# yassouali/pytorch-segmentation

Hardware: NVIDIA H100
Metric: images/sec DeepLabV3+/ResNet101 513x513 train step (fwd+CE+bwd+SGD) (higher is better)
Workload: dtype bf16

## Files before the change

include/seg_b200.h:

```cpp
#ifndef SEG_B200_H
#define SEG_B200_H

#include <stdint.h>

#ifdef __cplusplus
extern "C" {
#endif

#define SEG_DT_BF16 0
#define SEG_DT_F32 1

#define SEG_IMPL_AUTO 0
#define SEG_IMPL_SIMT 1
#define SEG_IMPL_TC 2

typedef struct seg_conv_desc {
  int32_t N, H, W, C;
  int32_t K;
  int32_t R, S;
  int32_t stride, pad, dil;
  int32_t P, Q;
  int32_t ldx;
  int32_t ldy;
} seg_conv_desc;

typedef struct seg_sync_desc {
  void* const* peers;
  int32_t rank, world, n_max;
  int64_t timeout_clocks;
} seg_sync_desc;

const char* seg_last_error(void);
int seg_version(void);
int seg_device_ok(void);
int64_t seg_launch_count(void);
void seg_launch_count_reset(void);

int seg_conv2d_fwd(const seg_conv_desc* d, const void* x, const void* w_packed, void* y, int y_dtype,
                   const float* bias, float beta, double* stats, const seg_sync_desc* sync, void* sync_ticket,
                   int impl, void* stream);
int seg_conv2d_dgrad(const seg_conv_desc* d, const void* dy, const void* w_packed, void* dx, float beta,
                     int impl, void* stream);
int64_t seg_conv2d_wgrad_workspace_floats(const seg_conv_desc* d, int impl);
int seg_conv2d_wgrad(const seg_conv_desc* d, const void* dy, const void* x, float* dw_packed, float* workspace, int impl,
                     void* stream);

int64_t seg_dwconv_scratch_floats(int C);
int seg_dwconv3x3_fwd(const seg_conv_desc* d, const void* x, const float* w9, void* y, double* stats,
                      const seg_sync_desc* sync, void* sync_ticket, void* stream);
int seg_dwconv3x3_bwd_data(const seg_conv_desc* d, const void* dy, const float* w9, void* dx, float beta, void* stream);
int seg_dwconv3x3_bwd_weight(const seg_conv_desc* d, const void* dy, const void* x, float* dw9, float beta,
                             float* scratch, void* stream);
int seg_dw_pack_weight(const float* w_c133, float* w9, int C, void* stream);
int seg_dw_unpack_wgrad(const float* g9, float* g_c133, int C, float beta, void* stream);

int seg_pack_weight(const float* w_oihw, void* w_packed, int K, int C, int R, int S, int Cpad, void* stream);
int seg_unpack_wgrad(const float* dw_packed, float* g_oihw, int K, int C, int R, int S, int Cpad, float beta,
                     void* stream);
int seg_pack_entry_bytes(void);
int seg_pack_weights_batched(const void* table, int n, int64_t total, void* stream);
int seg_unpack_wgrads_batched(const void* table, int n, int64_t total, float beta, void* stream);
int seg_im2col(const seg_conv_desc* d, const void* x, int x_nchw_f32, void* col, int Kpad, void* stream);

int seg_bn_stats(const void* x, int64_t M, int C, int ldx, double* stats, const seg_sync_desc* sync, void* sync_ticket,
                 void* stream);
// ... 161 lines not shown
```

pytorch-segmentation_b200/csrc/seg_api.cu:

```cuda
#include <stdarg.h>
#include "seg_common.cuh"

namespace seg {

static thread_local char g_err[1024] = "";
std::atomic<long long> g_launches{0};

void set_error(const char* fmt, ...) {
  va_list ap;
  va_start(ap, fmt);
  vsnprintf(g_err, sizeof(g_err), fmt, ap);
  va_end(ap);
}

namespace tc {
bool supported(const seg_conv_desc* d);
int conv_fwd(const seg_conv_desc* d, const void* x, const void* w, void* y, int y_dtype, const float* bias, float beta,
             double* stats, unsigned* stat_ticket, const seg_sync_desc* sync, cudaStream_t stream);
int conv_dgrad(const seg_conv_desc* d, const void* dy, const void* w, void* dx, float beta, cudaStream_t stream);
int conv_wgrad(const seg_conv_desc* d, const void* dy, const void* x, float* dw, float* ws, cudaStream_t stream);
int64_t wgrad_workspace_floats(const seg_conv_desc* d);
}
namespace simt {
int conv_fwd(const seg_conv_desc* d, const void* x, const void* w, void* y, int y_dtype, const float* bias, float beta,
             double* stats, unsigned* stat_ticket, const seg_sync_desc* sync, cudaStream_t stream);
int conv_dgrad(const seg_conv_desc* d, const void* dy, const void* w, void* dx, float beta, cudaStream_t stream);
int conv_wgrad(const seg_conv_desc* d, const void* dy, const void* x, float* dw, cudaStream_t stream);
}

static int check_desc(const seg_conv_desc* d) {
  SEG_REQUIRE(d != nullptr, "null conv descriptor");
  SEG_REQUIRE(d->N > 0 && d->H > 0 && d->W > 0 && d->C > 0 && d->K > 0 && d->R > 0 && d->S > 0, "bad conv dims");
  SEG_REQUIRE(d->stride >= 1 && d->dil >= 1 && d->pad >= 0, "bad conv stride/dil/pad");
  const int P = (d->H + 2 * d->pad - d->dil * (d->R - 1) - 1) / d->stride + 1;
  const int Q = (d->W + 2 * d->pad - d->dil * (d->S - 1) - 1) / d->stride + 1;
  SEG_REQUIRE(P == d->P && Q == d->Q, "conv output size mismatch: expected %dx%d got %dx%d", P, Q, d->P, d->Q);
  SEG_REQUIRE(d->ldx >= d->C && d->ldy >= d->K, "conv pitch smaller than channel count");
  return 0;
}

static bool tma_base_ok(const void* p) { return (reinterpret_cast<uintptr_t>(p) & 15) == 0; }

}

// ... 25 lines not shown
}

int seg_conv2d_fwd(const seg_conv_desc* d, const void* x, const void* w_packed, void* y, int y_dtype, const float* bias,
                   float beta, double* stats, const seg_sync_desc* sync, void* sync_ticket, int impl, void* stream) {
  if (check_desc(d)) return 1;
  SEG_REQUIRE(!sync || (stats && sync_ticket), "seg_conv2d_fwd: SyncBN needs stats and a zeroed ticket word");
  SEG_REQUIRE(!stats || beta == 0.f, "seg_conv2d_fwd: BatchNorm statistics need beta = 0 (got beta = %g)", (double)beta);
  const bool tc_ok = tc::supported(d) && tma_base_ok(x) && tma_base_ok(w_packed);
  unsigned* tk = reinterpret_cast<unsigned*>(sync_ticket);
  if (impl == SEG_IMPL_TC || (impl == SEG_IMPL_AUTO && tc_ok))
    return tc::conv_fwd(d, x, w_packed, y, y_dtype, bias, beta, stats, tk, sync, ST(stream));
  return simt::conv_fwd(d, x, w_packed, y, y_dtype, bias, beta, stats, tk, sync, ST(stream));
}

int seg_conv2d_dgrad(const seg_conv_desc* d, const void* dy, const void* w_packed, void* dx, float beta, int impl,
                     void* stream) {
  if (check_desc(d)) return 1;
  const bool tc_ok = tc::supported(d) && d->ldy % 8 == 0 && tma_base_ok(dy) && tma_base_ok(w_packed);
  if (impl == SEG_IMPL_TC || (impl == SEG_IMPL_AUTO && tc_ok))
    return tc::conv_dgrad(d, dy, w_packed, dx, beta, ST(stream));
  return simt::conv_dgrad(d, dy, w_packed, dx, beta, ST(stream));
}

static bool wgrad_on_tc(const seg_conv_desc* d, int impl) {
  return impl == SEG_IMPL_TC || (impl == SEG_IMPL_AUTO && tc::supported(d) && d->ldy % 8 == 0);
}

int64_t seg_conv2d_wgrad_workspace_floats(const seg_conv_desc* d, int impl) {
  if (check_desc(d)) return -1;
  return wgrad_on_tc(d, impl) ? tc::wgrad_workspace_floats(d) : 0;
}

int seg_conv2d_wgrad(const seg_conv_desc* d, const void* dy, const void* x, float* dw_packed, float* workspace, int impl,
                     void* stream) {
  if (check_desc(d)) return 1;
  if (wgrad_on_tc(d, impl) && (impl == SEG_IMPL_TC || (tma_base_ok(dy) && tma_base_ok(x))))
    return tc::conv_wgrad(d, dy, x, dw_packed, workspace, ST(stream));
  return simt::conv_wgrad(d, dy, x, dw_packed, ST(stream));
}

}
```

pytorch-segmentation_b200/csrc/seg_conv_tc.cu:

```cuda
#include <cuda.h>
#include <mutex>
#include <stdlib.h>
#include "seg_common.cuh"
#include "seg_ptx.cuh"
#include "seg_sync.cuh"

namespace seg {
namespace tc {

using namespace ptx;

constexpr int BM = 128;
constexpr int BK = 64;
constexpr int A_BYTES = BM * 128;
constexpr int KIND_KK = 0, KIND_KM = 1;
constexpr int NTHREADS = 384;
constexpr int NCONS = 256;
constexpr int MAXT = 49;

constexpr int BAR_CONSUMERS = 1;
constexpr int BAR_ORDER = 2;
constexpr int BAR_WG = 4;

struct TcParams {
  CUtensorMap mapA;
  CUtensorMap mapB;
  int M;
  int Ncols;
  int taps;
  int kchunks;
  int stride;
  int lower_h, lower_w;
  int PQ, Q;
  int x_im2col;
  int brows_per_tap;
  short tap_wt[MAXT];
  short tap_oh[MAXT];
  short tap_ow[MAXT];
  void* out;
  long long ldo;
  int out_dtype;
  float beta;
  const float* bias;
  double* stats;
  int stat_rows;
  unsigned* stat_ticket;
  SyncDesc sync;
  int out_strided, out_H, out_W, osy, osx, opy, opx;
  int n_tiles, tiles;
// ... 17 lines not shown
__device__ __forceinline__ void wgmma_tile(float* acc, uint64_t adesc, uint64_t bdesc, uint32_t accumulate) {
  if constexpr (BN == 64) wgmma_m64n64k16<TA, TB>(acc, adesc, bdesc, accumulate);
  else if constexpr (BN == 128) wgmma_m64n128k16<TA, TB>(acc, adesc, bdesc, accumulate);
  else wgmma_m64n256k16<TA, TB>(acc, adesc, bdesc, accumulate);
}

template <int BN, int KIND>
__device__ __forceinline__ void load_kblock(const TcParams& p, uint32_t a_dst, uint32_t bar, int kc, int wtap, uint16_t oh,
                                            uint16_t ow, int n_img, int h0, int w0, int m0, int n0) {
  const uint32_t b_dst = a_dst + A_BYTES;
  if (p.x_im2col)
    tma_load_im2col_4d(a_dst, &p.mapA, bar, kc * BK, w0, h0, n_img, ow, oh);
  else
    tma_load_2d(a_dst, &p.mapA, bar, kc * BK, m0);
  if (KIND == KIND_KK) {
    tma_load_2d(b_dst, &p.mapB, bar, kc * BK, wtap * p.brows_per_tap + n0);
  } else {
#pragma unroll
    for (int j = 0; j < BN / 64; ++j)
      tma_load_2d(b_dst + j * 8192, &p.mapB, bar, n0 + j * 64, wtap * p.brows_per_tap + kc * BK);
  }
}

template <int BN>
__device__ __forceinline__ void stage_acc(const float* acc, const float* acc1, uint8_t* stage, int rbase, int warp, int lane,
                                          const float* bias, bool out_f32) {
  const int esize = out_f32 ? 4 : 2;
  const int CPR = BN * esize / 16;
  const int swz = (CPR >= 32 ? 31 : CPR - 1);
  const int r0 = rbase + warp * 16 + (lane >> 2);
#pragma unroll
  for (int j = 0; j < BN / 8; ++j) {
    const int col = j * 8 + 2 * (lane & 3);
    float b0 = 0.f, b1 = 0.f;
    if (bias) {
      b0 = bias[col];
      b1 = bias[col + 1];
    }
#pragma unroll
    for (int h = 0; h < 4; ++h) {
      if (h >= 2 && !acc1) break;
      const float* a = h < 2 ? acc : acc1;
      const int r = r0 + 8 * (h & 1) + 32 * (h & 2);
      const float x0 = a[4 * j + 2 * (h & 1)] + b0, x1 = a[4 * j + 2 * (h & 1) + 1] + b1;
      const int byte = col * esize;
      uint8_t* dst = stage + (size_t)r * (BN * esize) + ((((byte >> 4) ^ (r & swz))) << 4) + (byte & 15);
      if (out_f32)
        *reinterpret_cast<float2*>(dst) = make_float2(x0, x1);
      else
        *reinterpret_cast<__nv_bfloat162*>(dst) = __floats2bfloat162_rn(x0, x1);
    }
  }
}


template <int BN, int ESIZE>
__device__ __forceinline__ void store_tile(const TcParams& p, const uint8_t* stage, int tid, int m0, int n0, int ncols_tile) {
  constexpr int CPR = BN * ESIZE / 16;
  constexpr int swz = (CPR >= 32 ? 31 : CPR - 1);
  constexpr int RSTEP = 128 / CPR;
  constexpr int NCH = BM / RSTEP;
  constexpr int BATCH = 8;
  static_assert(128 % CPR == 0 && NCH % BATCH == 0, "chunk walk of the staged tile");
  const int c16 = tid % CPR;
  const int nchunks = (ncols_tile * ESIZE + 15) >> 4;
  if (c16 >= nchunks) return;
  const bool vec_ok = ((p.ldo * ESIZE) & 15) == 0 && ((reinterpret_cast<uintptr_t>(p.out) + (size_t)n0 * ESIZE) & 15) == 0;
  const int first_col = (c16 << 4) / ESIZE;
  const bool full = first_col + 16 / ESIZE <= ncols_tile;
  auto row_dst = [&](int tr) {
    const int grow = m0 + tr;
    long long pixel = grow;
    if (p.out_strided) {
      const int n = grow / p.PQ;
      const int rem = grow - n * p.PQ;
      const int i = rem / p.Q, jj = rem - i * p.Q;
      pixel = ((long long)n * p.out_H + (i * p.osy + p.opy)) * p.out_W + (jj * p.osx + p.opx);
    }
    return reinterpret_cast<uint8_t*>(p.out) + ((size_t)pixel * p.ldo + n0) * ESIZE + ((size_t)c16 << 4);
  };
  auto row_src = [&](int tr) { return stage + (size_t)tr * (BN * ESIZE) + ((c16 ^ (tr & swz)) << 4); };
  if (ESIZE == 2 && vec_ok && full && p.beta != 0.f) {
    for (int b = 0; b < NCH; b += BATCH) {
      uint8_t* dst[BATCH];
      uint4 old[BATCH];
#pragma unroll
      for (int u = 0; u < BATCH; ++u) {
        const int tr = tid / CPR + (b + u) * RSTEP;
        dst[u] = m0 + tr < p.M ? row_dst(tr) : nullptr;
        old[u] = dst[u] ? *reinterpret_cast<const uint4*>(dst[u]) : make_uint4(0u, 0u, 0u, 0u);
      }
#pragma unroll
      for (int u = 0; u < BATCH; ++u) {
        if (!dst[u]) continue;
        float a[8], o[8];
        unpack8(*reinterpret_cast<const bf16x8*>(row_src(tid / CPR + (b + u) * RSTEP)), a);
        unpack8(*reinterpret_cast<const bf16x8*>(&old[u]), o);
#pragma unroll
        for (int k = 0; k < 8; ++k) a[k] += p.beta * o[k];
        *reinterpret_cast<bf16x8*>(dst[u]) = pack8(a);
      }
    }
    return;
  }
// ... 18 lines not shown
      const float a[4] = {val.x, val.y, val.z, val.w};
      float* d = reinterpret_cast<float*>(dst);
      if (vec_ok && full && p.beta == 0.f) {
        *reinterpret_cast<float4*>(d) = val;
      } else {
        for (int k = 0; k < 4; ++k)
          if (first_col + k < ncols_tile) d[k] = (p.beta != 0.f) ? a[k] + p.beta * d[k] : a[k];
      }
    }
  }
}

template <int BN>
struct PPCfg {
  static_assert(BN == 64 || BN == 128, "ping-pong tile width");
  static constexpr int B_BYTES = BN * 128;
  static constexpr int STAGE_BYTES = A_BYTES + B_BYTES;
  static constexpr int STAGES = BN == 64 ? 6 : 4;
  static constexpr int RING = STAGES * STAGE_BYTES;
  static constexpr int STG_BYTES = BM * 256;
  static constexpr int MAXG = BM / 32;
  static constexpr int STAT_BYTES = MAXG * 2 * BN * 4 + BN * 4;
  static constexpr int SMEM = RING + 2 * (STG_BYTES + STAT_BYTES) + 1024  + 256 ;
  static_assert(16 * STAGES + 8 <= 256, "barrier area");
  static_assert(SMEM <= 227 * 1024, "shared memory per block");
};

template <int BN, int KIND>
__global__ void __launch_bounds__(NTHREADS, 1) conv_gemm_pp(const __grid_constant__ TcParams p) {
  using C = PPCfg<BN>;
  constexpr int STAGES = C::STAGES;
  extern __shared__ uint8_t smem_raw[];
  const uint32_t raw_addr = smem_u32(smem_raw);
  const uint32_t smem0 = (raw_addr + 1023u) & ~1023u;
  uint8_t* smem_gen = smem_raw + (smem0 - raw_addr);
  const uint32_t bar0 = smem0 + C::RING + 2 * (C::STG_BYTES + C::STAT_BYTES);
  auto full_bar = [&](int s) { return bar0 + 8u * s; };
  auto empty_bar = [&](int s) { return bar0 + 8u * (STAGES + s); };
  volatile int* flag_sm = reinterpret_cast<volatile int*>(smem_gen + (bar0 - smem0) + 16 * STAGES);

  const int num_iters = p.taps * p.kchunks;
  const int grid = gridDim.x;
  const int ntiles = (p.tiles - (int)blockIdx.x + grid - 1) / grid;

  if (threadIdx.x == 0) {
    prefetch_tmap(&p.mapA);
    prefetch_tmap(&p.mapB);
    for (int s = 0; s < STAGES; ++s) {
      mbar_init(full_bar(s), 1);
      mbar_init(empty_bar(s), 4);
    }
    fence_mbar_init();
  }
  __syncthreads();
  pdl_wait();

  if (threadIdx.x < 128) {
    setmaxnreg_dec<40>();
    if (threadIdx.x == 0 && num_iters > 0) {
      int it = 0;
      for (int j = 0; j < ntiles; ++j) {
        const int t = blockIdx.x + j * grid;
        const int m0 = (t / p.n_tiles) * BM, n0 = (t % p.n_tiles) * BN;
        int n_img = 0, h0 = 0, w0 = 0;
        if (p.x_im2col) row_to_coords(m0, p.PQ, p.Q, p.stride, p.lower_h, p.lower_w, n_img, h0, w0);
        for (int tap = 0; tap < p.taps; ++tap) {
          const int wtap = p.tap_wt[tap];
          const uint16_t oh = (uint16_t)p.tap_oh[tap], ow = (uint16_t)p.tap_ow[tap];
          for (int kc = 0; kc < p.kchunks; ++kc, ++it) {
            const int st = it % STAGES;
            mbar_wait_nocall(empty_bar(st), ((it / STAGES) & 1) ^ 1u);
            mbar_arrive_expect_tx(full_bar(st), C::STAGE_BYTES);
            load_kblock<BN, KIND>(p, smem0 + st * C::STAGE_BYTES, full_bar(st), kc, wtap, oh, ow, n_img, h0, w0, m0, n0);
          }
        }
      }
    }
    return;
  }

  setmaxnreg_inc<232>();
  const int cw = (threadIdx.x - 128) >> 7;
  const int tid = threadIdx.x & 127;
  const int warp = tid >> 5, lane = tid & 31;
  uint8_t* stage = smem_gen + C::RING + cw * C::STG_BYTES;
  float* stat_sm = reinterpret_cast<float*>(smem_gen + C::RING + 2 * C::STG_BYTES + cw * C::STAT_BYTES);
  float* bias_sm = stat_sm + C::MAXG * 2 * BN;
  const bool out_f32 = p.out_dtype != SEG_DT_BF16;
  const int esize = out_f32 ? 4 : 2;
  const int CPR = BN * esize / 16;
  const int swz = (CPR >= 32 ? 31 : CPR - 1);
  auto wg_sync = [&] { named_sync(BAR_WG + cw, 128); };

  for (int j = cw; j < ntiles; j += 2) {
    const int t = blockIdx.x + j * grid;
    const int m0 = (t / p.n_tiles) * BM, n0 = (t % p.n_tiles) * BN;
    float acc0[BN / 2], acc1[BN / 2];
#pragma unroll
    for (int i = 0; i < BN / 2; ++i) acc0[i] = acc1[i] = 0.f;

    if (j > 0) named_sync(BAR_ORDER + cw, NCONS);
    {
      constexpr int TB = (KIND == KIND_KK) ? 0 : 1;
      const int it0 = j * num_iters;
      for (int i = 0; i < num_iters; ++i) {
        const int it = it0 + i;
        const int st = it % STAGES;
        mbar_wait_nocall(full_bar(st), (it / STAGES) & 1);
        const uint32_t a_addr = smem0 + st * C::STAGE_BYTES;
        const uint32_t b_addr = a_addr + A_BYTES;
        const uint64_t adesc0 = make_smem_desc_sw128(a_addr, 16, 1024);
        const uint64_t adesc1 = make_smem_desc_sw128(a_addr + 8192, 16, 1024);
        const uint64_t bdesc0 = make_smem_desc_sw128(b_addr, TB ? 8192 : 16, 1024);
        wgmma_fence();
#pragma unroll
        for (int k = 0; k < BK / 16; ++k) {
          const uint64_t bdesc = bdesc0 + (uint64_t)(TB ? (k * 2048 >> 4) : (k * 32 >> 4));
          wgmma_tile<BN, 0, TB>(acc0, adesc0 + (uint64_t)(k * 32 >> 4), bdesc, 1u);
          wgmma_tile<BN, 0, TB>(acc1, adesc1 + (uint64_t)(k * 32 >> 4), bdesc, 1u);
        }
        wgmma_commit();
        wgmma_wait<1>();
        __syncwarp();
        if (i > 0 && lane == 0) mbar_arrive(empty_bar((it - 1) % STAGES));
      }
      if (j + 1 < ntiles) named_arrive(BAR_ORDER + (cw ^ 1), NCONS);
      wgmma_wait<0>();
      __syncwarp();
      if (num_iters > 0 && lane == 0) mbar_arrive(empty_bar((it0 + num_iters - 1) % STAGES));
    }

    const int ncols_tile = min(BN, p.Ncols - n0);
    if (p.bias && tid < BN) bias_sm[tid] = tid < ncols_tile ? __ldg(p.bias + n0 + tid) : 0.f;
    wg_sync();
    stage_acc<BN>(acc0, acc1, stage, 0, warp, lane, p.bias ? bias_sm : nullptr, out_f32);
    wg_sync();

    const int ngroups = BM / p.stat_rows;
    if (p.stats) {
      const int parts = min(128 / BN, ngroups);
      const int rpp = BM / parts;
      const int c = tid % BN, part = tid / BN;
      const int rvalid = min(BM, p.M - m0);
      if (part < parts) {
        const int byte = c * esize;
        int g = part * rpp / p.stat_rows;
        auto load = [&](int r) {
          const uint8_t* src = stage + (size_t)r * (BN * esize) + ((((byte >> 4) ^ (r & swz))) << 4) + (byte & 15);
          return out_f32 ? *reinterpret_cast<const float*>(src) : bf2f(*reinterpret_cast<const __nv_bfloat16*>(src));
        };
        for (int rg = part * rpp; rg < (part + 1) * rpp; rg += p.stat_rows, ++g) {
          float s1 = 0.f, s2 = 0.f;
          const int rend = min(rg + p.stat_rows, rvalid);
          int r = rg;
          for (; r + 8 <= rend; r += 8) {
            float x[8];
#pragma unroll
            for (int u = 0; u < 8; ++u) x[u] = load(r + u);
#pragma unroll
            for (int u = 0; u < 8; ++u) {
              s1 += x[u];
              s2 = fmaf(x[u], x[u], s2);
            }
          }
          for (; r < rend; ++r) {
            const float x = load(r);
            s1 += x;
            s2 = fmaf(x, x, s2);
          }
          stat_sm[(g * 2 + 0) * BN + c] = s1;
          stat_sm[(g * 2 + 1) * BN + c] = s2;
        }
      }
    }

    if (out_f32)
      store_tile<BN, 4>(p, stage, tid, m0, n0, ncols_tile);
    else
      store_tile<BN, 2>(p, stage, tid, m0, n0, ncols_tile);
    if (j == ntiles - 1 && tid == 0) pdl_trigger();

    if (p.stats) {
      wg_sync();
      if (tid < ncols_tile) {
        float a = 0.f, b = 0.f;
        for (int g = 0; g < ngroups; ++g) {
          a += stat_sm[(g * 2 + 0) * BN + tid];
          b += stat_sm[(g * 2 + 1) * BN + tid];
        }
        atomicAdd(p.stats + n0 + tid, (double)a);
        atomicAdd(p.stats + p.Ncols + n0 + tid, (double)b);
      }
    }
  }

  if (p.stats && p.sync.world > 0)
    sync_push_when_last<false>(p.sync, p.stats, 2 * p.Ncols, p.stat_ticket, gridDim.x, threadIdx.x - 128, NCONS,
                               [] { named_sync(BAR_CONSUMERS, NCONS); }, flag_sm);
}


template <int BN>
struct Cfg {
  static constexpr int B_BYTES = BN * 128;
  static constexpr int STAGE_BYTES = A_BYTES + B_BYTES;
  static constexpr int STAGES = BN == 64 ? 6 : (BN == 128 ? 5 : 4);
  static constexpr int SMEM = STAGES * STAGE_BYTES + 1024  + 256 ;
  static_assert(STAGES * STAGE_BYTES >= BM * BN * 4, "staging tile must fit in the pipeline ring");
  static_assert(SMEM <= 227 * 1024, "shared memory per block");
};

template <int BN>
__global__ void __launch_bounds__(NTHREADS, 1) conv_gemm_wgrad(const __grid_constant__ TcParams p) {
  using C = Cfg<BN>;
  constexpr int STAGES = C::STAGES;
  extern __shared__ uint8_t smem_raw[];
  const uint32_t raw_addr = smem_u32(smem_raw);
// ... 61 lines not shown
#pragma unroll
  for (int i = 0; i < BN / 2; ++i) acc[i] = 0.f;
  for (int it = 0; it < num_iters; ++it) {
    const int st = it % STAGES;
    mbar_wait_nocall(full_bar(st), (it / STAGES) & 1);
    const uint32_t a_addr = smem0 + st * C::STAGE_BYTES + cw * 8192;
    const uint32_t b_addr = smem0 + st * C::STAGE_BYTES + A_BYTES;
    const uint64_t adesc0 = make_smem_desc_sw128(a_addr, 8192, 1024);
    const uint64_t bdesc0 = make_smem_desc_sw128(b_addr, 8192, 1024);
    wgmma_fence();
#pragma unroll
    for (int k = 0; k < BK / 16; ++k)
      wgmma_tile<BN, 1, 1>(acc, adesc0 + (uint64_t)(k * 2048 >> 4), bdesc0 + (uint64_t)(k * 2048 >> 4), 1u);
    wgmma_commit();
    wgmma_wait<1>();
    __syncwarp();
    if (it > 0 && lane == 0) mbar_arrive(empty_bar((it - 1) % STAGES));
  }
  wgmma_wait<0>();
  named_sync(BAR_CONSUMERS, NCONS);

  uint8_t* stage = smem_gen;
  const int ncols_tile = min(BN, p.Ncols - n0);
  stage_acc<BN>(acc, nullptr, stage, cw * 64, warp, lane, nullptr, true);
  named_sync(BAR_CONSUMERS, NCONS);

  const int CPR = BN * 4 / 16;
  const int swz = (CPR >= 32 ? 31 : CPR - 1);
  float* base = p.ws ? p.ws + (size_t)split * p.taps * p.dw_K * p.dw_C : p.dw;
  for (int idx = ctid; idx < BM * CPR; idx += NCONS) {
    const int tr = idx / CPR, c16 = idx - tr * CPR;
    const int row = m0 + tr, col0 = c16 * 4;
    if (row >= p.M || col0 >= ncols_tile) continue;
    const float4 v = *reinterpret_cast<const float4*>(stage + (size_t)tr * (BN * 4) + ((c16 ^ (tr & swz)) << 4));
    float* dst = base + ((size_t)tap_mm * p.dw_K + row) * p.dw_C + n0 + col0;
    const bool vec = col0 + 4 <= ncols_tile && ((reinterpret_cast<uintptr_t>(dst) & 15) == 0);
    const float a[4] = {v.x, v.y, v.z, v.w};
    if (p.ws) {
      if (vec)
        *reinterpret_cast<float4*>(dst) = v;
      else
        for (int i = 0; i < 4; ++i)
          if (col0 + i < ncols_tile) dst[i] = a[i];
    } else if (vec) {
      asm volatile("red.global.add.v4.f32 [%0], {%1, %2, %3, %4};" ::"l"(dst), "f"(v.x), "f"(v.y), "f"(v.z), "f"(v.w)
                   : "memory");
    } else {
      for (int i = 0; i < 4; ++i)
        if (col0 + i < ncols_tile) atomicAdd(dst + i, a[i]);
    }
  }
}

typedef CUresult (*EncodeTiledFn)(CUtensorMap*, CUtensorMapDataType, cuuint32_t, void*, const cuuint64_t*,
                                  const cuuint64_t*, const cuuint32_t*, const cuuint32_t*, CUtensorMapInterleave,
                                  CUtensorMapSwizzle, CUtensorMapL2promotion, CUtensorMapFloatOOBfill);
typedef CUresult (*EncodeIm2colFn)(CUtensorMap*, CUtensorMapDataType, cuuint32_t, void*, const cuuint64_t*,
// ... 43 lines not shown
  SEG_REQUIRE((reinterpret_cast<uintptr_t>(ptr) & 15) == 0, "TMA: base pointer not 16-byte aligned");
  SEG_REQUIRE(ld % 8 == 0, "TMA: channel pitch %lld not a multiple of 8", (long long)ld);
  SEG_REQUIRE(lower_w >= -128 && upper_w >= -128 && lower_w <= 127 && upper_w <= 127 && lower_h >= -128 &&
                  upper_h >= -128 && lower_h <= 127 && upper_h <= 127,
              "im2col corner out of range");
  cuuint64_t dims[4] = {(cuuint64_t)C, (cuuint64_t)W, (cuuint64_t)H, (cuuint64_t)N};
  cuuint64_t strides[3] = {(cuuint64_t)ld * 2, (cuuint64_t)W * ld * 2, (cuuint64_t)H * W * ld * 2};
  int lo[2] = {lower_w, lower_h};
  int up[2] = {upper_w, upper_h};
  cuuint32_t es[4] = {1, (cuuint32_t)stride, (cuuint32_t)stride, 1};
  CUresult r = g_encode_im2col(m, CU_TENSOR_MAP_DATA_TYPE_BFLOAT16, 4, const_cast<void*>(ptr), dims, strides, lo, up,
                               64, (cuuint32_t)pixels, es, CU_TENSOR_MAP_INTERLEAVE_NONE, CU_TENSOR_MAP_SWIZZLE_128B,
                               CU_TENSOR_MAP_L2_PROMOTION_L2_256B, CU_TENSOR_MAP_FLOAT_OOB_FILL_NONE);
  SEG_REQUIRE(r == CUDA_SUCCESS,
              "cuTensorMapEncodeIm2col failed (%d) N=%d H=%d W=%d C=%d ld=%lld lo=(%d,%d) up=(%d,%d) s=%d", (int)r, N, H,
              W, C, (long long)ld, lower_w, lower_h, upper_w, upper_h, stride);
  if (g_driver_version <= 13010) {
    const uint64_t bytes = (uint64_t)N * H * W * ld * 2;
    if (bytes < 131072) reinterpret_cast<uint64_t*>(m)[1] &= ~(1ull << 21);
  }
  return 0;
}

template <int BN, int KIND>
static int launch_pp(TcParams& p, cudaStream_t stream) {
  static bool attr_set = false;
  auto kfn = conv_gemm_pp<BN, KIND>;
  if (!attr_set) {
    cudaError_t e = cudaFuncSetAttribute(kfn, cudaFuncAttributeMaxDynamicSharedMemorySize, PPCfg<BN>::SMEM);
    SEG_REQUIRE(e == cudaSuccess, "cudaFuncSetAttribute(smem=%d): %s", PPCfg<BN>::SMEM, cudaGetErrorString(e));
    attr_set = true;
  }
  const int n_tiles = ceil_div(p.Ncols, BN);
  const int64_t tiles = ceil_div64(p.M, BM) * n_tiles;
  SEG_REQUIRE(tiles < (1ll << 31), "too many output tiles");
  p.n_tiles = n_tiles;
  p.tiles = (int)tiles;
  const dim3 grid((unsigned)std::min<int64_t>(tiles, num_sms()));
  launch_pdl(kfn, grid, dim3(NTHREADS), (size_t)PPCfg<BN>::SMEM, stream, p);
  return check_launch("conv_gemm_pp");
}

template <int KIND>
static int launch_pp_bn(int bn, TcParams& p, cudaStream_t stream) {
  switch (bn) {
    case 64: return launch_pp<64, KIND>(p, stream);
    case 128: return launch_pp<128, KIND>(p, stream);
  }
  set_error("bad BN %d", bn);
  return 1;
}

template <int BN>
static int launch_wgrad(const TcParams& p, dim3 grid, cudaStream_t stream) {
  static bool attr_set = false;
  auto kfn = conv_gemm_wgrad<BN>;
  if (!attr_set) {
    cudaError_t e = cudaFuncSetAttribute(kfn, cudaFuncAttributeMaxDynamicSharedMemorySize, Cfg<BN>::SMEM);
    SEG_REQUIRE(e == cudaSuccess, "cudaFuncSetAttribute(smem=%d): %s", Cfg<BN>::SMEM, cudaGetErrorString(e));
    attr_set = true;
  }
  launch_pdl(kfn, grid, dim3(NTHREADS), (size_t)Cfg<BN>::SMEM, stream, p);
// ... 234 lines not shown
```

pytorch-segmentation_b200/csrc/seg_ptx.cuh:

```cuda
#pragma once
#include <cuda.h>
#include <stdint.h>

namespace seg {
namespace ptx {

__device__ __forceinline__ uint32_t smem_u32(const void* p) { return (uint32_t)__cvta_generic_to_shared(p); }

__device__ __forceinline__ void mbar_init(uint32_t bar, uint32_t count) {
  asm volatile("mbarrier.init.shared::cta.b64 [%0], %1;" ::"r"(bar), "r"(count) : "memory");
}
__device__ __forceinline__ void fence_mbar_init() {
  asm volatile("fence.mbarrier_init.release.cluster;" ::: "memory");
}
__device__ __forceinline__ void fence_proxy_async() {
  asm volatile("fence.proxy.async.shared::cta;" ::: "memory");
}
__device__ __forceinline__ void mbar_arrive(uint32_t bar) {
  asm volatile("mbarrier.arrive.shared::cta.b64 _, [%0];" ::"r"(bar) : "memory");
}
__device__ __forceinline__ void mbar_arrive_expect_tx(uint32_t bar, uint32_t bytes) {
  asm volatile("mbarrier.arrive.expect_tx.shared::cta.b64 _, [%0], %1;" ::"r"(bar), "r"(bytes) : "memory");
}
__device__ __forceinline__ uint32_t mbar_try_wait(uint32_t bar, uint32_t parity) {
// ... 23 lines not shown
  if (mbar_try_wait(bar, parity)) return;
  long long t0 = clock64();
  while (!mbar_try_wait(bar, parity))
    if (clock64() - t0 > 4000000000ll) __trap();
}

__device__ __forceinline__ void prefetch_tmap(const CUtensorMap* m) {
  asm volatile("prefetch.tensormap [%0];" ::"l"(reinterpret_cast<uint64_t>(m)) : "memory");
}
__device__ __forceinline__ void tma_load_2d(uint32_t dst, const CUtensorMap* m, uint32_t bar, int c0, int c1) {
  asm volatile(
      "cp.async.bulk.tensor.2d.shared::cluster.global.mbarrier::complete_tx::bytes [%0], [%1, {%3, %4}], [%2];" ::"r"(dst),
      "l"(reinterpret_cast<uint64_t>(m)), "r"(bar), "r"(c0), "r"(c1)
      : "memory");
}
__device__ __forceinline__ void tma_load_im2col_4d(uint32_t dst, const CUtensorMap* m, uint32_t bar, int c, int w,
                                                   int h, int n, uint16_t off_w, uint16_t off_h) {
  asm volatile(
      "cp.async.bulk.tensor.4d.shared::cluster.global.im2col.mbarrier::complete_tx::bytes [%0], [%1, {%3, %4, %5, "
      "%6}], [%2], {%7, %8};" ::"r"(dst),
      "l"(reinterpret_cast<uint64_t>(m)), "r"(bar), "r"(c), "r"(w), "r"(h), "r"(n), "h"(off_w), "h"(off_h)
      : "memory");
}

template <int N>
__device__ __forceinline__ void setmaxnreg_inc() { asm volatile("setmaxnreg.inc.sync.aligned.u32 %0;" ::"n"(N)); }
template <int N>
__device__ __forceinline__ void setmaxnreg_dec() { asm volatile("setmaxnreg.dec.sync.aligned.u32 %0;" ::"n"(N)); }
__device__ __forceinline__ void named_sync(int id, int count) {
  asm volatile("bar.sync %0, %1;" ::"r"(id), "r"(count) : "memory");
}
__device__ __forceinline__ void named_arrive(int id, int count) {
  asm volatile("bar.arrive %0, %1;" ::"r"(id), "r"(count) : "memory");
}

__device__ __forceinline__ void wgmma_fence() { asm volatile("wgmma.fence.sync.aligned;" ::: "memory"); }
__device__ __forceinline__ void wgmma_commit() { asm volatile("wgmma.commit_group.sync.aligned;" ::: "memory"); }
template <int N>
__device__ __forceinline__ void wgmma_wait() { asm volatile("wgmma.wait_group.sync.aligned %0;" ::"n"(N) : "memory"); }

__device__ __forceinline__ uint64_t make_smem_desc_sw128(uint32_t smem_addr, uint32_t lbo_bytes, uint32_t sbo_bytes) {
  uint64_t d = 0;
  d |= (uint64_t)((smem_addr & 0x3FFFFu) >> 4);
  d |= (uint64_t)((lbo_bytes >> 4) & 0x3FFFu) << 16;
  d |= (uint64_t)((sbo_bytes >> 4) & 0x3FFFu) << 32;
  d |= (uint64_t)1 << 62;
// ... 39 lines not shown
```

pytorch-segmentation_b200/seg_b200/lib.py:

```python
import ctypes
import os
from ctypes import POINTER, Structure, c_char_p, c_double, c_float, c_int, c_int32, c_int64, c_uint8, c_uint32, c_uint64, c_void_p

import torch

_HERE = os.path.dirname(os.path.abspath(__file__))
LIB_PATH = os.path.join(os.path.dirname(_HERE), "libseg_b200.so")

DT_BF16, DT_F32 = 0, 1
IMPL_AUTO, IMPL_SIMT, IMPL_TC = 0, 1, 2
LOSS_CE, LOSS_WCE, LOSS_FOCAL = 0, 1, 2


class SyncDesc(Structure):

    _fields_ = [("peers", c_void_p), ("rank", c_int32), ("world", c_int32), ("n_max", c_int32), ("timeout_clocks", c_int64)]


class ConvDesc(Structure):

    _fields_ = [(n, c_int32) for n in ("N", "H", "W", "C", "K", "R", "S", "stride", "pad", "dil", "P", "Q", "ldx", "ldy")]


def conv_out_size(size, k, stride, pad, dil):
    return (size + 2 * pad - dil * (k - 1) - 1) // stride + 1


def make_conv_desc(N, H, W, C, K, R, S, stride, pad, dil, ldx=None, ldy=None):
    P = conv_out_size(H, R, stride, pad, dil)
    Q = conv_out_size(W, S, stride, pad, dil)
    return ConvDesc(N, H, W, C, K, R, S, stride, pad, dil, P, Q, ldx if ldx is not None else C, ldy if ldy is not None else K)


_SIGS = {
    "seg_last_error": (c_char_p, []),
    "seg_version": (c_int, []),
    "seg_device_ok": (c_int, []),
    "seg_launch_count": (c_int64, []),
    "seg_launch_count_reset": (None, []),
    "seg_conv2d_fwd": (c_int, [POINTER(ConvDesc), c_void_p, c_void_p, c_void_p, c_int, c_void_p, c_float, c_void_p, c_void_p, c_void_p, c_int, c_void_p]),
    "seg_conv2d_dgrad": (c_int, [POINTER(ConvDesc), c_void_p, c_void_p, c_void_p, c_float, c_int, c_void_p]),
    "seg_conv2d_wgrad_workspace_floats": (c_int64, [POINTER(ConvDesc), c_int]),
    "seg_conv2d_wgrad": (c_int, [POINTER(ConvDesc), c_void_p, c_void_p, c_void_p, c_void_p, c_int, c_void_p]),
    "seg_dwconv_scratch_floats": (c_int64, [c_int]),
    "seg_dwconv3x3_fwd": (c_int, [POINTER(ConvDesc), c_void_p, c_void_p, c_void_p, c_void_p, c_void_p, c_void_p, c_void_p]),
    "seg_dwconv3x3_bwd_data": (c_int, [POINTER(ConvDesc), c_void_p, c_void_p, c_void_p, c_float, c_void_p]),
    "seg_dwconv3x3_bwd_weight": (c_int, [POINTER(ConvDesc), c_void_p, c_void_p, c_void_p, c_float, c_void_p, c_void_p]),
    "seg_dw_pack_weight": (c_int, [c_void_p, c_void_p, c_int, c_void_p]),
    "seg_dw_unpack_wgrad": (c_int, [c_void_p, c_void_p, c_int, c_float, c_void_p]),
    "seg_pack_weight": (c_int, [c_void_p, c_void_p, c_int, c_int, c_int, c_int, c_int, c_void_p]),
    "seg_unpack_wgrad": (c_int, [c_void_p, c_void_p, c_int, c_int, c_int, c_int, c_int, c_float, c_void_p]),
    "seg_pack_entry_bytes": (c_int, []),
    "seg_pack_weights_batched": (c_int, [c_void_p, c_int, c_int64, c_void_p]),
    "seg_unpack_wgrads_batched": (c_int, [c_void_p, c_int, c_int64, c_float, c_void_p]),
    "seg_im2col": (c_int, [POINTER(ConvDesc), c_void_p, c_int, c_void_p, c_int, c_void_p]),
    "seg_bn_stats": (c_int, [c_void_p, c_int64, c_int, c_int, c_void_p, c_void_p, c_void_p, c_void_p]),
    "seg_bn_finalize": (c_int, [c_void_p, c_double, c_int, c_void_p, c_void_p, c_float, c_float, c_int, c_void_p, c_void_p, c_void_p, c_void_p, c_void_p]),
    "seg_bn_eval_scale_shift": (c_int, [c_int, c_void_p, c_void_p, c_void_p, c_void_p, c_float, c_void_p, c_void_p, c_void_p]),
    "seg_bn_apply": (c_int, [c_void_p, c_int, c_void_p, c_void_p, c_int, c_void_p, c_int, c_int64, c_int, c_int, c_float, c_uint64, c_void_p, c_int, c_void_p]),
    "seg_counter_add": (c_int, [c_void_p, c_uint64, c_void_p]),
    "seg_bn_bwd_reduce_slots": (c_int, []),
    "seg_bn_bwd_reduce": (c_int, [c_void_p, c_int, c_void_p, c_int, c_void_p, c_int, c_void_p, c_int64, c_int, c_int, c_float, c_void_p, c_void_p, c_void_p, c_void_p, c_void_p, c_int, c_void_p, c_void_p, c_void_p, c_void_p]),
    "seg_bn_apply_train": (c_int, [c_void_p, c_int, c_void_p, c_double, c_void_p, c_void_p, c_float, c_float, c_int, c_void_p, c_void_p, c_void_p, c_void_p, c_int, c_void_p, c_int, c_int64, c_int, c_int, c_float, c_uint64, c_void_p, c_int, c_void_p]),
    "seg_bn_bwd_fused_workspace": (c_int, [c_int64, c_int, POINTER(c_int64), POINTER(c_int64)]),
# ... 123 lines not shown
```

pytorch-segmentation_b200/seg_b200/ops.py:

```python
import ctypes

import torch

from . import lib
from .lib import DT_BF16, DT_F32, IMPL_AUTO, IMPL_SIMT, IMPL_TC, ConvDesc, call, make_conv_desc, ptr

_IMPL_OVERRIDE = None
PROFILE = None


def _meta(d):
    if lib.TRACE is None:
        return None
    return (d.N, d.H, d.W, d.C, d.K, d.R, d.stride, d.dil, 2.0 * d.N * d.P * d.Q * d.K * d.C * d.R * d.S)


def _meta_rows(M, C, passes, flag=0):
    if lib.TRACE is None:
        return None
    return (int(M), int(C), int(flag), 0, 0, 0, 0, 0, 2.0 * M * C * passes)


def _prof(kind, d):
    if PROFILE is None:
# ... 82 lines not shown
    assert stats is None or stats.dtype == torch.float64
    sp, tp, _keep = _sync_args(sync if stats is not None else None, sync_ticket, x.device)
    ev = _prof("fprop", d)
    call("seg_conv2d_fwd", ctypes.byref(d), ptr(x), ptr(w_packed), ptr(out), DT_BF16 if out.dtype == torch.bfloat16 else DT_F32,
         ptr(bias), float(beta), ptr(stats), sp, tp, _impl(impl), meta=_meta(d))
    if ev is not None:
        ev.record()
    return out


def conv2d_dgrad(dy, w_packed, x_shape, R, S, stride=1, pad=0, dil=1, out=None, beta=0.0, impl=IMPL_AUTO):
    N, H, W, C = x_shape
    K = dy.shape[-1]
    if out is None:
        out = torch.empty((N, H, W, C), dtype=torch.bfloat16, device=dy.device)
        beta = 0.0
    d = make_conv_desc(N, H, W, C, K, R, S, stride, pad, dil, ldx=ld(out), ldy=ld(dy))
    assert (d.P, d.Q) == (dy.shape[1], dy.shape[2])
    ev = _prof("dgrad", d)
    call("seg_conv2d_dgrad", ctypes.byref(d), ptr(dy), ptr(w_packed), ptr(out), float(beta), _impl(impl), meta=_meta(d))
    if ev is not None:
        ev.record()
    return out


def conv2d_wgrad(dy, x, R, S, stride=1, pad=0, dil=1, out=None, impl=IMPL_AUTO):
    N, H, W, C = x.shape
    K = dy.shape[-1]
    if out is None:
        out = torch.zeros((R * S, K, C), dtype=torch.float32, device=x.device)
    d = make_conv_desc(N, H, W, C, K, R, S, stride, pad, dil, ldx=ld(x), ldy=ld(dy))
    assert (d.P, d.Q) == (dy.shape[1], dy.shape[2])
    nws = lib.load().seg_conv2d_wgrad_workspace_floats(ctypes.byref(d), _impl(impl))
    if nws < 0:
        raise RuntimeError(f"seg_conv2d_wgrad_workspace_floats failed: {lib.last_error()}")
    ws = torch.empty(nws, dtype=torch.float32, device=x.device) if nws > 0 else None
    ev = _prof("wgrad", d)
    call("seg_conv2d_wgrad", ctypes.byref(d), ptr(dy), ptr(x), ptr(out), ptr(ws), _impl(impl), meta=_meta(d))
    if ev is not None:
        ev.record()
    return out


def dw_pack_weight(w_c133):
    C = w_c133.shape[0]
    w9 = torch.empty((9, C), dtype=torch.float32, device=w_c133.device)
# ... 544 lines not shown
```

Measured before the change: 371.1.

## Store conv GEMM output tiles via TMA bulk stores with swizzled staging

Conv forward and dgrad epilogues now write the staged output tile to global memory with TMA 2D bulk stores instead of per-thread vector stores. The staging layout changes to 128B-swizzled slices so it matches the tensor map. When beta is nonzero, the old output tile is prefetched by TMA load into the stage and blended in registers. This is meant to cut epilogue store instruction overhead and let stores overlap the next tile's mainloop, at the cost of extra tensor-map encoding per launch and new bulk-group synchronization.

```diff
diff --git a/include/seg_b200.h b/include/seg_b200.h
--- a/include/seg_b200.h
+++ b/include/seg_b200.h
@@ -41,6 +41,7 @@
                    int impl, void* stream);
 int seg_conv2d_dgrad(const seg_conv_desc* d, const void* dy, const void* w_packed, void* dx, float beta,
                      int impl, void* stream);
+int seg_conv2d_out_route(const seg_conv_desc* d, int dgrad, const void* out, int out_dtype, float beta);
 int64_t seg_conv2d_wgrad_workspace_floats(const seg_conv_desc* d, int impl);
 int seg_conv2d_wgrad(const seg_conv_desc* d, const void* dy, const void* x, float* dw_packed, float* workspace, int impl,
                      void* stream);
diff --git a/pytorch-segmentation_b200/csrc/seg_api.cu b/pytorch-segmentation_b200/csrc/seg_api.cu
--- a/pytorch-segmentation_b200/csrc/seg_api.cu
+++ b/pytorch-segmentation_b200/csrc/seg_api.cu
@@ -20,6 +20,7 @@
 int conv_dgrad(const seg_conv_desc* d, const void* dy, const void* w, void* dx, float beta, cudaStream_t stream);
 int conv_wgrad(const seg_conv_desc* d, const void* dy, const void* x, float* dw, float* ws, cudaStream_t stream);
 int64_t wgrad_workspace_floats(const seg_conv_desc* d);
+int conv_out_route(const seg_conv_desc* d, int dgrad, const void* out, int out_dtype, float beta);
 }
 namespace simt {
 int conv_fwd(const seg_conv_desc* d, const void* x, const void* w, void* y, int y_dtype, const float* bias, float beta,
@@ -91,6 +92,11 @@
   return simt::conv_dgrad(d, dy, w_packed, dx, beta, ST(stream));
 }
 
+int seg_conv2d_out_route(const seg_conv_desc* d, int dgrad, const void* out, int out_dtype, float beta) {
+  if (check_desc(d)) return -1;
+  return tc::conv_out_route(d, dgrad, out, out_dtype, beta);
+}
+
 static bool wgrad_on_tc(const seg_conv_desc* d, int impl) {
   return impl == SEG_IMPL_TC || (impl == SEG_IMPL_AUTO && tc::supported(d) && d->ldy % 8 == 0);
 }
diff --git a/pytorch-segmentation_b200/csrc/seg_conv_tc.cu b/pytorch-segmentation_b200/csrc/seg_conv_tc.cu
--- a/pytorch-segmentation_b200/csrc/seg_conv_tc.cu
+++ b/pytorch-segmentation_b200/csrc/seg_conv_tc.cu
@@ -22,9 +22,14 @@
 constexpr int BAR_ORDER = 2;
 constexpr int BAR_WG = 4;
 
+constexpr int ROUTE_STORES = 0;
+constexpr int ROUTE_TMA = 1;
+constexpr int ROUTE_TMA_OLD = 2;
+
 struct TcParams {
   CUtensorMap mapA;
   CUtensorMap mapB;
+  CUtensorMap mapO;
   int M;
   int Ncols;
   int taps;
@@ -88,13 +93,17 @@
   }
 }
 
+__device__ __forceinline__ int stage_off_sw(int r, int byte, int sw) {
+  return (byte >> 7) * (BM * 128) + r * 128 + ((((byte >> 4) & 7) ^ sw) << 4) + (byte & 15);
+}
+__device__ __forceinline__ int stage_off(int r, int byte) { return stage_off_sw(r, byte, r & 7); }
+
 template <int BN>
 __device__ __forceinline__ void stage_acc(const float* acc, const float* acc1, uint8_t* stage, int rbase, int warp, int lane,
-                                          const float* bias, bool out_f32) {
+                                          const float* bias, bool out_f32, float beta) {
   const int esize = out_f32 ? 4 : 2;
-  const int CPR = BN * esize / 16;
-  const int swz = (CPR >= 32 ? 31 : CPR - 1);
   const int r0 = rbase + warp * 16 + (lane >> 2);
+  const int sw = r0 & 7;
 #pragma unroll
   for (int j = 0; j < BN / 8; ++j) {
     const int col = j * 8 + 2 * (lane & 3);
@@ -109,12 +118,23 @@
       const float* a = h < 2 ? acc : acc1;
       const int r = r0 + 8 * (h & 1) + 32 * (h & 2);
       const float x0 = a[4 * j + 2 * (h & 1)] + b0, x1 = a[4 * j + 2 * (h & 1) + 1] + b1;
-      const int byte = col * esize;
-      uint8_t* dst = stage + (size_t)r * (BN * esize) + ((((byte >> 4) ^ (r & swz))) << 4) + (byte & 15);
-      if (out_f32)
-        *reinterpret_cast<float2*>(dst) = make_float2(x0, x1);
-      else
-        *reinterpret_cast<__nv_bfloat162*>(dst) = __floats2bfloat162_rn(x0, x1);
+      uint8_t* dst = stage + stage_off_sw(r, col * esize, sw);
+      if (out_f32) {
+        float2 v = make_float2(x0, x1);
+        if (beta != 0.f) {
+          const float2 o = *reinterpret_cast<const float2*>(dst);
+          v = make_float2(fmaf(beta, o.x, v.x), fmaf(beta, o.y, v.y));
+        }
+        *reinterpret_cast<float2*>(dst) = v;
+      } else {
+        __nv_bfloat162 v = __floats2bfloat162_rn(x0, x1);
+        if (beta != 0.f) {
+          const float2 o = __bfloat1622float2(*reinterpret_cast<const __nv_bfloat162*>(dst));
+          const float2 f = __bfloat1622float2(v);
+          v = __floats2bfloat162_rn(fmaf(beta, o.x, f.x), fmaf(beta, o.y, f.y));
+        }
+        *reinterpret_cast<__nv_bfloat162*>(dst) = v;
+      }
     }
   }
 }
@@ -123,7 +143,6 @@
 template <int BN, int ESIZE>
 __device__ __forceinline__ void store_tile(const TcParams& p, const uint8_t* stage, int tid, int m0, int n0, int ncols_tile) {
   constexpr int CPR = BN * ESIZE / 16;
-  constexpr int swz = (CPR >= 32 ? 31 : CPR - 1);
   constexpr int RSTEP = 128 / CPR;
   constexpr int NCH = BM / RSTEP;
   constexpr int BATCH = 8;
@@ -145,7 +164,7 @@
     }
     return reinterpret_cast<uint8_t*>(p.out) + ((size_t)pixel * p.ldo + n0) * ESIZE + ((size_t)c16 << 4);
   };
-  auto row_src = [&](int tr) { return stage + (size_t)tr * (BN * ESIZE) + ((c16 ^ (tr & swz)) << 4); };
+  auto row_src = [&](int tr) { return stage + stage_off(tr, c16 << 4); };
   if (ESIZE == 2 && vec_ok && full && p.beta != 0.f) {
     for (int b = 0; b < NCH; b += BATCH) {
       uint8_t* dst[BATCH];
@@ -210,11 +229,11 @@
   static constexpr int MAXG = BM / 32;
   static constexpr int STAT_BYTES = MAXG * 2 * BN * 4 + BN * 4;
   static constexpr int SMEM = RING + 2 * (STG_BYTES + STAT_BYTES) + 1024  + 256 ;
-  static_assert(16 * STAGES + 8 <= 256, "barrier area");
+  static_assert(16 * STAGES + 8 + 16 <= 256, "barrier area: ring barriers, SyncBN flag, one old-tile barrier per consumer");
   static_assert(SMEM <= 227 * 1024, "shared memory per block");
 };
 
-template <int BN, int KIND>
+template <int BN, int KIND, int ROUTE>
 __global__ void __launch_bounds__(NTHREADS, 1) conv_gemm_pp(const __grid_constant__ TcParams p) {
   using C = PPCfg<BN>;
   constexpr int STAGES = C::STAGES;
@@ -226,6 +245,7 @@
   auto full_bar = [&](int s) { return bar0 + 8u * s; };
   auto empty_bar = [&](int s) { return bar0 + 8u * (STAGES + s); };
   volatile int* flag_sm = reinterpret_cast<volatile int*>(smem_gen + (bar0 - smem0) + 16 * STAGES);
+  auto old_bar = [&](int c) { return bar0 + 16u * STAGES + 8u + 8u * c; };
 
   const int num_iters = p.taps * p.kchunks;
   const int grid = gridDim.x;
@@ -234,10 +254,13 @@
   if (threadIdx.x == 0) {
     prefetch_tmap(&p.mapA);
     prefetch_tmap(&p.mapB);
+    if (ROUTE != ROUTE_STORES) prefetch_tmap(&p.mapO);
     for (int s = 0; s < STAGES; ++s) {
       mbar_init(full_bar(s), 1);
       mbar_init(empty_bar(s), 4);
     }
+    mbar_init(old_bar(0), 1);
+    mbar_init(old_bar(1), 1);
     fence_mbar_init();
   }
   __syncthreads();
@@ -276,16 +299,25 @@
   float* bias_sm = stat_sm + C::MAXG * 2 * BN;
   const bool out_f32 = p.out_dtype != SEG_DT_BF16;
   const int esize = out_f32 ? 4 : 2;
-  const int CPR = BN * esize / 16;
-  const int swz = (CPR >= 32 ? 31 : CPR - 1);
+  constexpr int route = ROUTE;
+  const uint32_t stage_u32 = smem0 + C::RING + cw * C::STG_BYTES;
+  constexpr uint32_t SLICE = BM * 128;
   auto wg_sync = [&] { named_sync(BAR_WG + cw, 128); };
 
   for (int j = cw; j < ntiles; j += 2) {
     const int t = blockIdx.x + j * grid;
     const int m0 = (t / p.n_tiles) * BM, n0 = (t % p.n_tiles) * BN;
+    const int ncols_tile = min(BN, p.Ncols - n0);
+    const int nbox = (ncols_tile * esize + 127) >> 7;
     float acc0[BN / 2], acc1[BN / 2];
 #pragma unroll
     for (int i = 0; i < BN / 2; ++i) acc0[i] = acc1[i] = 0.f;
+
+    if (route == ROUTE_TMA_OLD && tid == 0) {
+      bulk_wait_read<0>();
+      mbar_arrive_expect_tx(old_bar(cw), nbox * SLICE);
+      for (int b = 0; b < nbox; ++b) tma_load_2d(stage_u32 + b * SLICE, &p.mapO, old_bar(cw), n0 + b * (128 / esize), m0);
+    }
 
     if (j > 0) named_sync(BAR_ORDER + cw, NCONS);
     {
@@ -318,11 +350,19 @@
       if (num_iters > 0 && lane == 0) mbar_arrive(empty_bar((it0 + num_iters - 1) % STAGES));
     }
 
-    const int ncols_tile = min(BN, p.Ncols - n0);
     if (p.bias && tid < BN) bias_sm[tid] = tid < ncols_tile ? __ldg(p.bias + n0 + tid) : 0.f;
+    if (route != ROUTE_STORES && tid == 0) bulk_wait_read<0>();
     wg_sync();
-    stage_acc<BN>(acc0, acc1, stage, 0, warp, lane, p.bias ? bias_sm : nullptr, out_f32);
+    if (route == ROUTE_TMA_OLD) mbar_wait_nocall(old_bar(cw), (j >> 1) & 1);
+    stage_acc<BN>(acc0, acc1, stage, 0, warp, lane, p.bias ? bias_sm : nullptr, out_f32,
+                  route == ROUTE_TMA_OLD ? p.beta : 0.f);
+    if (route != ROUTE_STORES) fence_proxy_async();
     wg_sync();
+
+    if (route != ROUTE_STORES && tid == 0) {
+      for (int b = 0; b < nbox; ++b) tma_store_2d(&p.mapO, stage_u32 + b * SLICE, n0 + b * (128 / esize), m0);
+      bulk_commit();
+    }
 
     const int ngroups = BM / p.stat_rows;
     if (p.stats) {
@@ -333,24 +373,28 @@
       if (part < parts) {
         const int byte = c * esize;
         int g = part * rpp / p.stat_rows;
-        auto load = [&](int r) {
-          const uint8_t* src = stage + (size_t)r * (BN * esize) + ((((byte >> 4) ^ (r & swz))) << 4) + (byte & 15);
+        auto value = [&](const uint8_t* src) {
           return out_f32 ? *reinterpret_cast<const float*>(src) : bf2f(*reinterpret_cast<const __nv_bfloat16*>(src));
         };
+        int off8[8];
+#pragma unroll
+        for (int u = 0; u < 8; ++u) off8[u] = stage_off_sw(u, byte, u);
         for (int rg = part * rpp; rg < (part + 1) * rpp; rg += p.stat_rows, ++g) {
           float s1 = 0.f, s2 = 0.f;
           const int rend = min(rg + p.stat_rows, rvalid);
           int r = rg;
           for (; r + 8 <= rend; r += 8) {
+            const uint8_t* rowp = stage + r * 128;
             float x[8];
 #pragma unroll
-            for (int u = 0; u < 8; ++u) x[u] = load(r + u);
+            for (int u = 0; u < 8; ++u) x[u] = value(rowp + off8[u]);
 #pragma unroll
             for (int u = 0; u < 8; ++u) {
               s1 += x[u];
               s2 = fmaf(x[u], x[u], s2);
             }
           }
+          auto load = [&](int r) { return value(stage + stage_off(r, byte)); };
           for (; r < rend; ++r) {
             const float x = load(r);
             s1 += x;
@@ -362,10 +406,12 @@
       }
     }
 
-    if (out_f32)
-      store_tile<BN, 4>(p, stage, tid, m0, n0, ncols_tile);
-    else
-      store_tile<BN, 2>(p, stage, tid, m0, n0, ncols_tile);
+    if (route == ROUTE_STORES) {
+      if (out_f32)
+        store_tile<BN, 4>(p, stage, tid, m0, n0, ncols_tile);
+      else
+        store_tile<BN, 2>(p, stage, tid, m0, n0, ncols_tile);
+    }
     if (j == ntiles - 1 && tid == 0) pdl_trigger();
 
     if (p.stats) {
@@ -381,6 +427,7 @@
       }
     }
   }
+  if (route != ROUTE_STORES && tid == 0) bulk_wait<0>();
 
   if (p.stats && p.sync.world > 0)
     sync_push_when_last<false>(p.sync, p.stats, 2 * p.Ncols, p.stat_ticket, gridDim.x, threadIdx.x - 128, NCONS,
@@ -488,17 +535,16 @@
 
   uint8_t* stage = smem_gen;
   const int ncols_tile = min(BN, p.Ncols - n0);
-  stage_acc<BN>(acc, nullptr, stage, cw * 64, warp, lane, nullptr, true);
+  stage_acc<BN>(acc, nullptr, stage, cw * 64, warp, lane, nullptr, true, 0.f);
   named_sync(BAR_CONSUMERS, NCONS);
 
   const int CPR = BN * 4 / 16;
-  const int swz = (CPR >= 32 ? 31 : CPR - 1);
   float* base = p.ws ? p.ws + (size_t)split * p.taps * p.dw_K * p.dw_C : p.dw;
   for (int idx = ctid; idx < BM * CPR; idx += NCONS) {
     const int tr = idx / CPR, c16 = idx - tr * CPR;
     const int row = m0 + tr, col0 = c16 * 4;
     if (row >= p.M || col0 >= ncols_tile) continue;
-    const float4 v = *reinterpret_cast<const float4*>(stage + (size_t)tr * (BN * 4) + ((c16 ^ (tr & swz)) << 4));
+    const float4 v = *reinterpret_cast<const float4*>(stage + stage_off(tr, c16 << 4));
     float* dst = base + ((size_t)tap_mm * p.dw_K + row) * p.dw_C + n0 + col0;
     const bool vec = col0 + 4 <= ncols_tile && ((reinterpret_cast<uintptr_t>(dst) & 15) == 0);
     const float a[4] = {v.x, v.y, v.z, v.w};
@@ -588,13 +634,43 @@
   return 0;
 }
 
+static int make_map_out(CUtensorMap* m, void* ptr, int64_t rows, int64_t cols, int64_t ld, bool f32) {
+  if (resolve_driver()) return 1;
+  const int esize = f32 ? 4 : 2;
+  cuuint64_t dims[2] = {(cuuint64_t)cols, (cuuint64_t)rows};
+  cuuint64_t strides[1] = {(cuuint64_t)(ld * esize)};
+  cuuint32_t box[2] = {(cuuint32_t)(128 / esize), (cuuint32_t)BM};
+  cuuint32_t es[2] = {1, 1};
+  CUresult r = g_encode_tiled(m, f32 ? CU_TENSOR_MAP_DATA_TYPE_FLOAT32 : CU_TENSOR_MAP_DATA_TYPE_BFLOAT16, 2, ptr, dims,
+                              strides, box, es, CU_TENSOR_MAP_INTERLEAVE_NONE, CU_TENSOR_MAP_SWIZZLE_128B,
+                              CU_TENSOR_MAP_L2_PROMOTION_L2_256B, CU_TENSOR_MAP_FLOAT_OOB_FILL_NONE);
+  SEG_REQUIRE(r == CUDA_SUCCESS, "cuTensorMapEncodeTiled (output) failed (%d) rows=%lld cols=%lld ld=%lld f32=%d", (int)r,
+              (long long)rows, (long long)cols, (long long)ld, (int)f32);
+  return 0;
+}
+
+static int out_route(const void* out, long long ldo, int ncols, int esize, bool strided, int taps, float beta) {
+  if (strided || taps == 0 || (reinterpret_cast<uintptr_t>(out) & 15) != 0 || (ldo * esize) % 16 != 0 ||
+      (ncols * esize) % 16 != 0)
+    return ROUTE_STORES;
+  return beta != 0.f ? ROUTE_TMA_OLD : ROUTE_TMA;
+}
+
+int conv_out_route(const seg_conv_desc* d, int dgrad, const void* out, int out_dtype, float beta) {
+  if (dgrad) return out_route(out, d->ldx, d->C, 2, d->stride > 1, d->R * d->S, beta);
+  return out_route(out, d->ldy, d->K, out_dtype == SEG_DT_BF16 ? 2 : 4, false, d->R * d->S, beta);
+}
+
 template <int BN, int KIND>
 static int launch_pp(TcParams& p, cudaStream_t stream) {
   static bool attr_set = false;
-  auto kfn = conv_gemm_pp<BN, KIND>;
+  void (*const kfns[3])(TcParams) = {conv_gemm_pp<BN, KIND, ROUTE_STORES>, conv_gemm_pp<BN, KIND, ROUTE_TMA>,
+                                     conv_gemm_pp<BN, KIND, ROUTE_TMA_OLD>};
   if (!attr_set) {
-    cudaError_t e = cudaFuncSetAttribute(kfn, cudaFuncAttributeMaxDynamicSharedMemorySize, PPCfg<BN>::SMEM);
-    SEG_REQUIRE(e == cudaSuccess, "cudaFuncSetAttribute(smem=%d): %s", PPCfg<BN>::SMEM, cudaGetErrorString(e));
+    for (auto kfn : kfns) {
+      cudaError_t e = cudaFuncSetAttribute(kfn, cudaFuncAttributeMaxDynamicSharedMemorySize, PPCfg<BN>::SMEM);
+      SEG_REQUIRE(e == cudaSuccess, "cudaFuncSetAttribute(smem=%d): %s", PPCfg<BN>::SMEM, cudaGetErrorString(e));
+    }
     attr_set = true;
   }
   const int n_tiles = ceil_div(p.Ncols, BN);
@@ -602,8 +678,11 @@
   SEG_REQUIRE(tiles < (1ll << 31), "too many output tiles");
   p.n_tiles = n_tiles;
   p.tiles = (int)tiles;
+  const bool f32 = p.out_dtype != SEG_DT_BF16;
+  const int route = out_route(p.out, p.ldo, p.Ncols, f32 ? 4 : 2, p.out_strided, p.taps, p.beta);
+  if (route != ROUTE_STORES && make_map_out(&p.mapO, p.out, p.M, p.Ncols, p.ldo, f32)) return 1;
   const dim3 grid((unsigned)std::min<int64_t>(tiles, num_sms()));
-  launch_pdl(kfn, grid, dim3(NTHREADS), (size_t)PPCfg<BN>::SMEM, stream, p);
+  launch_pdl(kfns[route], grid, dim3(NTHREADS), (size_t)PPCfg<BN>::SMEM, stream, p);
   return check_launch("conv_gemm_pp");
 }
 
diff --git a/pytorch-segmentation_b200/csrc/seg_ptx.cuh b/pytorch-segmentation_b200/csrc/seg_ptx.cuh
--- a/pytorch-segmentation_b200/csrc/seg_ptx.cuh
+++ b/pytorch-segmentation_b200/csrc/seg_ptx.cuh
@@ -69,6 +69,17 @@
       "l"(reinterpret_cast<uint64_t>(m)), "r"(bar), "r"(c), "r"(w), "r"(h), "r"(n), "h"(off_w), "h"(off_h)
       : "memory");
 }
+__device__ __forceinline__ void tma_store_2d(const CUtensorMap* m, uint32_t src, int c0, int c1) {
+  asm volatile("cp.async.bulk.tensor.2d.global.shared::cta.bulk_group [%0, {%2, %3}], [%1];" ::"l"(
+                   reinterpret_cast<uint64_t>(m)),
+               "r"(src), "r"(c0), "r"(c1)
+               : "memory");
+}
+__device__ __forceinline__ void bulk_commit() { asm volatile("cp.async.bulk.commit_group;" ::: "memory"); }
+template <int N>
+__device__ __forceinline__ void bulk_wait_read() { asm volatile("cp.async.bulk.wait_group.read %0;" ::"n"(N) : "memory"); }
+template <int N>
+__device__ __forceinline__ void bulk_wait() { asm volatile("cp.async.bulk.wait_group %0;" ::"n"(N) : "memory"); }
 
 template <int N>
 __device__ __forceinline__ void setmaxnreg_inc() { asm volatile("setmaxnreg.inc.sync.aligned.u32 %0;" ::"n"(N)); }
diff --git a/pytorch-segmentation_b200/seg_b200/lib.py b/pytorch-segmentation_b200/seg_b200/lib.py
--- a/pytorch-segmentation_b200/seg_b200/lib.py
+++ b/pytorch-segmentation_b200/seg_b200/lib.py
@@ -40,6 +40,7 @@
     "seg_launch_count_reset": (None, []),
     "seg_conv2d_fwd": (c_int, [POINTER(ConvDesc), c_void_p, c_void_p, c_void_p, c_int, c_void_p, c_float, c_void_p, c_void_p, c_void_p, c_int, c_void_p]),
     "seg_conv2d_dgrad": (c_int, [POINTER(ConvDesc), c_void_p, c_void_p, c_void_p, c_float, c_int, c_void_p]),
+    "seg_conv2d_out_route": (c_int, [POINTER(ConvDesc), c_int, c_void_p, c_int, c_float]),
     "seg_conv2d_wgrad_workspace_floats": (c_int64, [POINTER(ConvDesc), c_int]),
     "seg_conv2d_wgrad": (c_int, [POINTER(ConvDesc), c_void_p, c_void_p, c_void_p, c_void_p, c_int, c_void_p]),
     "seg_dwconv_scratch_floats": (c_int64, [c_int]),
diff --git a/pytorch-segmentation_b200/seg_b200/ops.py b/pytorch-segmentation_b200/seg_b200/ops.py
--- a/pytorch-segmentation_b200/seg_b200/ops.py
+++ b/pytorch-segmentation_b200/seg_b200/ops.py
@@ -128,6 +128,20 @@
     if ev is not None:
         ev.record()
     return out
+
+
+ROUTE_STORES, ROUTE_TMA, ROUTE_TMA_OLD = 0, 1, 2
+
+
+def conv2d_out_route(dgrad, x_shape, K, R, S, out, stride=1, pad=0, dil=1, beta=0.0):
+    N, H, W, C = x_shape
+    pitch = ld(out)
+    d = make_conv_desc(N, H, W, C, K, R, S, stride, pad, dil, ldx=pitch if dgrad else C, ldy=K if dgrad else pitch)
+    r = lib.load().seg_conv2d_out_route(ctypes.byref(d), int(bool(dgrad)), ptr(out),
+                                        DT_BF16 if out.dtype == torch.bfloat16 else DT_F32, float(beta))
+    if r < 0:
+        raise RuntimeError(f"seg_conv2d_out_route failed: {lib.last_error()}")
+    return r
 
 
 def conv2d_wgrad(dy, x, R, S, stride=1, pad=0, dil=1, out=None, impl=IMPL_AUTO):
```

After: 381.3, median of 6. +2.7%, better.
